# LarissaReames-NOAA/MPASSIT

Hardware: AMD Instinct MI355X
Metric: interpolated 3-D fields/sec (nCells x nLev -> nx x ny) (higher is better)
Workload: dtype f64

## Files before the change

mpassit_amd/build.py:

```python
import os
import subprocess
import sys
from concurrent.futures import ThreadPoolExecutor

HERE = os.path.dirname(os.path.abspath(__file__))
CSRC = os.path.join(HERE, "csrc")
OBJDIR = os.path.join(HERE, "_build")
SO = os.path.join(HERE, "libmpassit_amd.so")
SOURCES = ["mpg_api.hip", "mpg_comm.hip", "mpg_hostpipe.hip", "mpg_fileio.hip", "k_setup.hip", "k_mesh_window.hip", "k_target_grid.hip", "k_store_bilinear.hip", "k_store_nearest.hip", "k_store_conserve.hip",
           "k_store_gridbil.hip", "k_apply.hip", "k_apply_lfu.hip", "k_apply_typed.hip", "k_wind.hip", "k_pole.hip", "k_post.hip", "k_halo.hip", "k_prims.hip", "k_sort.hip", "k_transpose.hip", "k_apply_masked.hip", "k_store_to_mesh.hip", "k_apply_to_mesh.hip", "k_apply_csr_to_mesh.hip", "k_store_mesh.hip", "k_apply_rows.hip",
           "k_store_conserve_mesh.hip", "k_apply_csr_rows.hip", "k_store_periodic_to_mesh.hip"]
HEADERS = ["mpg_internal.h", "geom.h", "quad_solve.h", "conserve_clip.h", "apply_mesh.h", os.path.join("..", "..", "include", "mpassit_amd.h")]
HIPCC = os.environ.get("HIPCC", "/opt/rocm/bin/hipcc")
FLAGS = ["--offload-arch=gfx950", "-O3", "-fPIC", "-std=c++17", "-Wall", "-Wno-unused-function", "-fno-gpu-rdc"]


def _newer(a, deps):
    if not os.path.exists(a):
        return False
    t = os.path.getmtime(a)
    return all(os.path.getmtime(d) <= t for d in deps)


def build(force=False, verbose=False):
    os.makedirs(OBJDIR, exist_ok=True)
    hdrs = [os.path.join(CSRC, h) for h in HEADERS]
    jobs = []
    objs = []
    for s in SOURCES:
        src = os.path.join(CSRC, s)
        obj = os.path.join(OBJDIR, s.replace(".hip", ".o"))
        objs.append(obj)
        if force or not _newer(obj, [src] + hdrs):
            jobs.append([HIPCC] + FLAGS + ["-c", src, "-o", obj])

    def run(cmd):
        if verbose:
            print(" ".join(cmd), flush=True)
        r = subprocess.run(cmd, capture_output=True, text=True)
        if r.returncode != 0:
            raise RuntimeError("hipcc failed:\n%s\n%s" % (" ".join(cmd), r.stderr[-8000:]))
        return r.stderr

    if jobs:
        with ThreadPoolExecutor(max_workers=min(4, len(jobs))) as ex:
# ... 102 lines not shown
```

mpassit_amd/csrc/mpg_api.hip:

```cpp
#include <stdarg.h>
#include <stdio.h>
#include <stdlib.h>
#include <string.h>
#include <time.h>

#include <condition_variable>
#include <deque>
#include <map>
#include <memory>
#include <mutex>
#include <thread>
#include <unordered_map>
#include <vector>

#include "mpg_internal.h"

static thread_local char g_err[1024] = "";
static bool g_init = false;
static int g_device = -1;
static hipStream_t g_stream = nullptr;
static std::map<HandleKey, mpg_handle_s *> g_cache;
#define MPG_MAX_PARKED 8
static uint64_t g_park_clock = 0;
static std::recursive_mutex g_cache_mu;
#define CACHE_LOCK() std::lock_guard<std::recursive_mutex> cache_lock_(g_cache_mu)
static void store_worker_drain();
static void store_worker_stop();
static int store_worker_start(int device);

void mpg_set_error(const char *fmt, ...) {
  va_list ap;
  va_start(ap, fmt);
  vsnprintf(g_err, sizeof(g_err), fmt, ap);
  va_end(ap);
}
bool mpg_is_initialized() { return g_init; }
hipStream_t mpg_setup_stream() { return g_stream; }
int mpg_device_index() { return g_device; }

void mpg_cache_detach(mpg_handle_s *h) {
  CACHE_LOCK();
  if (h->cached) {
    g_cache.erase(h->key);
    h->cached = false;
  }
}

namespace {
struct PoolBlock { void *p; size_t bytes; hipStream_t stream; };
std::vector<PoolBlock> g_pool;
std::mutex g_pool_mu;
size_t g_pool_bytes = 0;
const size_t POOL_CAP_BYTES = (size_t)4 << 30;
}

void *mpg_pool_get(size_t bytes, hipStream_t s) {
  bytes = (bytes + 255) & ~(size_t)255;
  {
    std::lock_guard<std::mutex> lk(g_pool_mu);
    int best = -1;
    for (int i = 0; i < (int)g_pool.size(); ++i) {
      const PoolBlock &b = g_pool[i];
      if (b.stream != s || b.bytes < bytes || b.bytes > 2 * bytes + (1 << 20)) continue;
      if (best < 0 || b.bytes < g_pool[best].bytes) best = i;
    }
    if (best >= 0) {
      void *p = g_pool[best].p;
      g_pool_bytes -= g_pool[best].bytes;
      g_pool.erase(g_pool.begin() + best);
      return p;
    }
  }
  void *p = nullptr;
  hipError_t e = hipMalloc(&p, bytes);
  if (e != hipSuccess) {
    mpg_pool_release();
    e = hipMalloc(&p, bytes);
  }
  if (e != hipSuccess) {
    mpg_set_error("HIP error %s allocating %zu bytes of scratch", hipGetErrorString(e), bytes);
    return nullptr;
  }
  return p;
}

static std::unordered_map<void *, size_t> g_pool_real;

void mpg_pool_put(void *p, size_t bytes, hipStream_t s) {
  if (!p) return;
  bytes = (bytes + 255) & ~(size_t)255;
  std::lock_guard<std::mutex> lk(g_pool_mu);
  auto it = g_pool_real.find(p);
  if (it != g_pool_real.end()) bytes = it->second;
  else g_pool_real[p] = bytes;
  if (g_pool_bytes + bytes > POOL_CAP_BYTES) {
    g_pool_real.erase(p);
    (void)hipFree(p);
    return;
  }
  g_pool.push_back(PoolBlock{p, bytes, s});
  g_pool_bytes += bytes;
}

void mpg_pool_release() {
  std::lock_guard<std::mutex> lk(g_pool_mu);
  for (const PoolBlock &b : g_pool) (void)hipFree(b.p);
  g_pool.clear();
  g_pool_real.clear();
  g_pool_bytes = 0;
}


#define MPG_ANCHORS(X) X(k_setup) X(k_target_grid) X(k_store_bilinear) X(k_store_nearest) X(k_store_conserve) X(k_store_gridbil) \
  X(k_apply) X(k_apply_lfu) X(k_apply_typed) X(k_wind) X(k_pole) X(k_post) X(k_halo) X(mpg_comm) X(k_mesh_window) X(k_prims) X(k_sort) \
  X(k_transpose) X(k_apply_masked) X(k_store_to_mesh) X(k_apply_to_mesh) X(k_apply_csr_to_mesh) \
  X(k_store_mesh) X(k_apply_rows) X(k_store_conserve_mesh) X(k_apply_csr_rows) X(k_store_periodic_to_mesh)
#define X(n) const void *mpg_anchor_##n();
MPG_ANCHORS(X)
#undef X
static std::thread *g_warm = nullptr;
static bool g_init_trace = false;
static double now_ms() {
  struct timespec ts;
  clock_gettime(CLOCK_MONOTONIC, &ts);
  return (double)ts.tv_sec * 1e3 + (double)ts.tv_nsec * 1e-6;
}
static void warm_modules(int device) {
  if (hipSetDevice(device) != hipSuccess) return;
  (void)store_worker_start(device);
  hipFuncAttributes a;
  double t0 = now_ms();
#define X(n)                                                                                                          \
  (void)hipFuncGetAttributes(&a, mpg_anchor_##n());                                                                   \
  if (g_init_trace) {                                                                                                 \
// ... 52 lines not shown
  MPG_ARG(device >= 0 && device < n, "mpg_init: device index out of range");
  if (g_init && device != g_device) {
    mpg_set_error("mpg_init: already initialised on device %d; call mpg_finalize before initialising device %d", g_device, device);
    return MPG_ERR_INVALID_ARG;
  }
  MPG_HIP(hipSetDevice(device));
  const double t_2 = now_ms();
  if (!g_init) {
    MPG_HIP(hipStreamCreateWithFlags(&g_stream, hipStreamNonBlocking));
    if (g_init_trace)
      fprintf(stderr, "mpg_init trace: hipGetDeviceCount (runtime start) %.2f ms, hipSetDevice %.2f ms, stream %.2f ms\n", t_1 - t_0, t_2 - t_1,
              now_ms() - t_2);
    const char *e = getenv("MPG_NO_WARMUP");
    if (!(e && *e == '1')) {
      g_warm = new std::thread(warm_modules, device);
      static bool registered = false;
      if (!registered) {
        atexit(warm_join);
        registered = true;
      }
    }
  }
  g_device = device;
  g_init = true;
  return MPG_SUCCESS;
}

int mpg_warmup_wait(void) {
  warm_join();
  store_worker_drain();
  return MPG_SUCCESS;
}

static void handle_free(mpg_handle_s *h);
static void drop_parked(void *obj) {
  CACHE_LOCK();
  for (auto it = g_cache.begin(); it != g_cache.end();) {
    mpg_handle_s *h = it->second;
    if (h->refcount == 0 && (!obj || std::get<0>(it->first) == obj || std::get<2>(it->first) == obj)) {
      it = g_cache.erase(it);
      handle_free(h);
    } else {
      ++it;
    }
  }
}

int mpg_finalize(void) {
  if (!g_init) return MPG_SUCCESS;
  warm_join();
  store_worker_stop();
  drop_parked(nullptr);
  mpg_fileio_release();
  mpg_hostpipe_release();
  (void)hipStreamSynchronize(g_stream);
  mpg_pool_release();
  (void)hipStreamDestroy(g_stream);
  g_stream = nullptr;
  g_init = false;
  return MPG_SUCCESS;
}

int mpg_device_count(int *n) {
  MPG_ARG(n, "mpg_device_count: NULL argument");
  int c = 0;
  if (hipGetDeviceCount(&c) != hipSuccess) c = 0;
// ... 7 lines not shown
  MPG_HIP(hipGetDeviceProperties(&p, g_device));
  if (arch_buf && buf_len > 0) {
    strncpy(arch_buf, p.gcnArchName, (size_t)buf_len - 1);
    arch_buf[buf_len - 1] = 0;
  }
  if (n_cu) *n_cu = p.multiProcessorCount;
  if (hbm_bytes) *hbm_bytes = (int64_t)p.totalGlobalMem;
  return MPG_SUCCESS;
}

static std::vector<mpg_mesh_s *> g_meshes;

static int mesh_common_checks(int64_t nCells, int64_t nVertices, int maxEdges, const double *latCell, const double *lonCell, const double *latVertex,
                              const double *lonVertex, const int32_t *verticesOnCell, mpg_mesh *out, const char *who) {
  if (!out) { mpg_set_error("%s: out is NULL", who); return MPG_ERR_INVALID_ARG; }
  if (!(nCells > 0 && nVertices > 0 && maxEdges >= 3)) { mpg_set_error("%s: nCells, nVertices must be > 0 and maxEdges >= 3", who); return MPG_ERR_INVALID_ARG; }
  if (!(nCells < 0x7fffffff && nVertices < 0x7fffffff)) { mpg_set_error("%s: sizes must fit int32 ids", who); return MPG_ERR_INVALID_ARG; }
  if (!(latCell && lonCell && latVertex && lonVertex && verticesOnCell)) { mpg_set_error("%s: NULL array", who); return MPG_ERR_INVALID_ARG; }
  return MPG_SUCCESS;
}

int mpg_mesh_create_window(int64_t nCells, int64_t nVertices, int maxEdges, const double *latCell, const double *lonCell, const double *latVertex,
                           const double *lonVertex, const int32_t *verticesOnCell, mpg_grid grid, mpg_mesh *out) {
  MPG_CHECK_INIT();
  int rc = mesh_common_checks(nCells, nVertices, maxEdges, latCell, lonCell, latVertex, lonVertex, verticesOnCell, out, "mpg_mesh_create_window");
  if (rc) return rc;
  MPG_ARG(grid, "mpg_mesh_create_window: NULL grid");
  mpg_mesh_s *m = new mpg_mesh_s();
  m->nCells = nCells;
  m->nVertices = nVertices;
  m->maxEdges = maxEdges;
  m->geo_grid = grid;
  g_meshes.push_back(m);
  if ((rc = mpg_k_mesh_coords(nCells, lonCell, latCell, m->cell, g_stream)) ||
      (rc = mpg_k_mesh_window(m, grid, latVertex, lonVertex, verticesOnCell, g_stream))) {
    mpg_mesh_destroy(m);
    return rc;
  }
  *out = m;
  return MPG_SUCCESS;
}

int mpg_mesh_window_info(mpg_mesh m, int64_t *cell_first, int64_t *cell_count, int64_t *vertex_first, int64_t *vertex_count, double *margin) {
  MPG_ARG(m, "mpg_mesh_window_info: NULL mesh");
  if (cell_first) *cell_first = m->cw0;
  if (cell_count) *cell_count = m->cwn;
  if (vertex_first) *vertex_first = m->vw0;
  if (vertex_count) *vertex_count = m->vwn;
  if (margin) *margin = m->geo_margin;
  return MPG_SUCCESS;
}

int mpg_mesh_create(int64_t nCells, int64_t nVertices, int maxEdges, const double *latCell, const double *lonCell,
                    const double *latVertex, const double *lonVertex, const int32_t *verticesOnCell, mpg_mesh *out) {
  MPG_CHECK_INIT();
  {
    int rc0 = mesh_common_checks(nCells, nVertices, maxEdges, latCell, lonCell, latVertex, lonVertex, verticesOnCell, out, "mpg_mesh_create");
    if (rc0) return rc0;
  }
  mpg_mesh_s *m = new mpg_mesh_s();
  m->nCells = nCells;
  m->nVertices = nVertices;
  m->maxEdges = maxEdges;
  m->cwn = nCells;
  m->vwn = nVertices;
  m->geo_margin = 4.0;
// ... 199 lines not shown
int mpg_grid_get_rotang(mpg_grid g, double *cosa_host, double *sina_host) {
  const double *c, *s;
  int rc = mpg_grid_rotang_dev(g, &c, &s);
  if (rc) return rc;
  size_t bytes = sizeof(double) * (size_t)g->nx * g->ny;
  if (cosa_host) MPG_HIP(hipMemcpy(cosa_host, c, bytes, hipMemcpyDeviceToHost));
  if (sina_host) MPG_HIP(hipMemcpy(sina_host, s, bytes, hipMemcpyDeviceToHost));
  return MPG_SUCCESS;
}

static void handle_free(mpg_handle_s *h) {
  h->idx.free();
  h->w.free();
  h->rowptr.free();
  h->col.free();
  h->val.free();
  h->dst_frac.free();
  h->pole_dst.free();
  h->pole_src0.free();
  h->pole_w.free();
  h->free_tile_lists();
  delete h;
}

struct StoreCtx {
  mpg_mesh_s *m;
  mpg_grid_s *g;
  int stagger;
  int method;
  int meshloc;
  mpg_mesh_s *dst_mesh = nullptr;
};

struct StoreJob {
  HandleKey key;
  int (*build)(mpg_handle_s *, void *, hipStream_t);
  StoreCtx ctx;
  hipEvent_t ready = nullptr;
  bool done = false;
  int rc = MPG_SUCCESS;
  char err[1024] = "";
  ~StoreJob() {
    if (ready) (void)hipEventDestroy(ready);
  }
};
struct StoreWorker {
  std::mutex mu, start_mu;
  std::condition_variable cv;
  std::deque<std::shared_ptr<StoreJob>> queue;
  std::map<HandleKey, std::shared_ptr<StoreJob>> pending;
  std::thread *thread = nullptr;
  hipStream_t stream = nullptr;
  bool stop = false;
};
static StoreWorker &SW() {
  static StoreWorker *w = new StoreWorker();
  return *w;
}
static const char *mpg_last_error_cstr() { return g_err; }

static int store_build_now(StoreJob &job, hipStream_t s) {
  mpg_handle_s *h = new mpg_handle_s();
  h->refcount = 0;
  hipEvent_t e0 = nullptr, e1 = nullptr;
  if (hipEventCreate(&e0) != hipSuccess || hipEventCreate(&e1) != hipSuccess) {
    mpg_set_error("hipEventCreate failed in a RegridStore");
    handle_free(h);
    return MPG_ERR_HIP;
  }
  (void)hipEventRecord(e0, s);
  int rc = job.build(h, &job.ctx, s);
  if (!rc) {
    hipError_t e = hipEventRecord(e1, s);
    if (e == hipSuccess) e = hipEventSynchronize(e1);
    if (e == hipSuccess) e = hipEventElapsedTime(&h->store_ms, e0, e1);
    if (e != hipSuccess) {
      mpg_set_error("RegridStore: %s", hipGetErrorString(e));
      rc = MPG_ERR_HIP;
    }
  }
  (void)hipEventDestroy(e0);
  (void)hipEventDestroy(e1);
  if (rc) {
    handle_free(h);
    return rc;
  }
  CACHE_LOCK();
  h->key = job.key;
  h->cached = true;
  h->parked_at = ++g_park_clock;
  g_cache[job.key] = h;
  return MPG_SUCCESS;
}

static void store_worker_main(int device) {
  const hipError_t dev_err = hipSetDevice(device);
  for (;;) {
    std::shared_ptr<StoreJob> job;
    {
      std::unique_lock<std::mutex> lk(SW().mu);
      SW().cv.wait(lk, [] { return SW().stop || !SW().queue.empty(); });
      if (SW().queue.empty()) return;
      job = SW().queue.front();
      SW().queue.pop_front();
    }
    g_err[0] = 0;
    int rc;
    if (dev_err != hipSuccess) {
      mpg_set_error("RegridStore: the Store worker could not bind device %d: %s", device, hipGetErrorString(dev_err));
      rc = MPG_ERR_HIP;
    } else {
      if (job->ready) (void)hipStreamWaitEvent(SW().stream, job->ready, 0);
      rc = store_build_now(*job, SW().stream);
    }
    {
      std::lock_guard<std::mutex> lk(SW().mu);
      job->rc = rc;
      if (rc) snprintf(job->err, sizeof(job->err), "%s", mpg_last_error_cstr());
      job->done = true;
      SW().pending.erase(job->key);
    }
    SW().cv.notify_all();
  }
}

static int store_worker_start(int device) {
  std::lock_guard<std::mutex> lk(SW().start_mu);
  if (SW().thread) return MPG_SUCCESS;
  MPG_HIP(hipStreamCreateWithFlags(&SW().stream, hipStreamNonBlocking));
  SW().stop = false;
  SW().thread = new std::thread(store_worker_main, device);
  return MPG_SUCCESS;
}

static void store_worker_drain() {
  std::unique_lock<std::mutex> lk(SW().mu);
  SW().cv.wait(lk, [] { return SW().pending.empty(); });
}

static void store_worker_stop() {
  if (!SW().thread) return;
  store_worker_drain();
  {
    std::lock_guard<std::mutex> lk(SW().mu);
    SW().stop = true;
  }
  SW().cv.notify_all();
  SW().thread->join();
  delete SW().thread;
  SW().thread = nullptr;
  (void)hipStreamDestroy(SW().stream);
  SW().stream = nullptr;
}

static int store_common(HandleKey key, mpg_handle *out, int (*build)(mpg_handle_s *, void *, hipStream_t), const StoreCtx &ctx) {
  for (int attempt = 0; attempt < 2; ++attempt) {
    {
      CACHE_LOCK();
      auto it = g_cache.find(key);
      if (it != g_cache.end()) {
        if (out) {
          it->second->refcount++;
          *out = it->second;
        }
        return MPG_SUCCESS;
      }
    }
    int rc = store_worker_start(g_device);
    if (rc) return rc;
    std::shared_ptr<StoreJob> job;
    {
      std::unique_lock<std::mutex> lk(SW().mu);
      auto pit = SW().pending.find(key);
      if (pit != SW().pending.end()) {
        job = pit->second;
      } else {
        job = std::make_shared<StoreJob>();
        job->key = key;
        job->build = build;
        job->ctx = ctx;
        if (hipEventCreateWithFlags(&job->ready, hipEventDisableTiming) == hipSuccess) (void)hipEventRecord(job->ready, g_stream);
        SW().pending[key] = job;
        SW().queue.push_back(job);
      }
      if (!out) {
        lk.unlock();
        SW().cv.notify_all();
        return MPG_SUCCESS;
      }
      SW().cv.notify_all();
      SW().cv.wait(lk, [&] { return job->done; });
    }
    if (job->rc) {
      mpg_set_error("%s", job->err);
      return job->rc;
    }
  }
  mpg_set_error("RegridStore: the finished handle left the cache before it was collected");
  return MPG_ERR_HIP;
}

static int store_mesh_build(mpg_handle_s *h, void *c, hipStream_t s) {
  StoreCtx *x = (StoreCtx *)c;
  h->method = x->method;
  int rc;
  if (x->method == MPG_REGRIDMETHOD_BILINEAR) rc = mpg_k_store_bilinear_mesh(x->m, x->g, x->stagger, x->meshloc, h, s);
  else if (x->method == MPG_REGRIDMETHOD_NEAREST_STOD) rc = mpg_k_store_nearest(x->m, x->g, x->stagger, h, s);
  else rc = mpg_k_store_conserve(x->m, x->g, h, s);
  if (!rc && x->m->win_count[x->meshloc] >= 0)
    rc = mpg_k_rebase(h, x->m->win_first[x->meshloc], x->m->win_count[x->meshloc], s, true);
  return rc;
}
static int store_grid_build(mpg_handle_s *h, void *c, hipStream_t s) {
  StoreCtx *x = (StoreCtx *)c;
  h->method = x->method;
  return mpg_k_store_grid_bilinear(x->g, x->stagger, h, s);
}

static int store_mesh_entry(mpg_mesh src, int src_meshloc, mpg_grid dst, int dst_staggerloc, int regridmethod, mpg_handle *out, const char *who) {
  MPG_CHECK_INIT();
  MPG_ARG(src && dst, "mpg_regrid_store: NULL argument");
  MPG_ARG(dst_staggerloc >= 0 && dst_staggerloc <= 2, "mpg_regrid_store: destination stagger must be CENTER, EDGE1 or EDGE2");
  MPG_ARG(src_meshloc == MPG_MESHLOC_ELEMENT || src_meshloc == MPG_MESHLOC_NODE, "mpg_regrid_store: unknown mesh location");
  if (src_meshloc == MPG_MESHLOC_NODE && regridmethod != MPG_REGRIDMETHOD_BILINEAR) {
    mpg_set_error("%s: node-located sources are only regridded bilinearly by the reference (interp.F90:350-366)", who);
    return MPG_ERR_UNSUPPORTED;
  }
  MPG_ARG(regridmethod >= 0 && regridmethod <= 2, "mpg_regrid_store: unknown regrid method");
  if (src->geo_grid && (src->geo_grid != dst || src->geo_grid_gone)) {
    mpg_set_error("%s: the mesh was cut to another grid (mpg_mesh_create_window%s); it holds only the cells that grid can see", who,
                  src->geo_grid_gone ? ", which has been destroyed" : "");
    return MPG_ERR_INVALID_ARG;
  }
  if (regridmethod == MPG_REGRIDMETHOD_CONSERVE && dst_staggerloc != MPG_STAGGERLOC_CENTER) {
    mpg_set_error("%s: conservative regridding is defined on the CENTER stagger only", who);
    return MPG_ERR_UNSUPPORTED;
  }
  StoreCtx ctx{src, dst, dst_staggerloc, regridmethod, src_meshloc};
  HandleKey key(src, src_meshloc, dst, dst_staggerloc,
                regridmethod + (regridmethod == MPG_REGRIDMETHOD_BILINEAR ? 16 * mpg_bilinear_linetype() : 0) +
                    (regridmethod == MPG_REGRIDMETHOD_BILINEAR && src_meshloc == MPG_MESHLOC_NODE ? 256 * (mpg_node_fan_origin() + 16) : 0));
  return store_common(key, out, store_mesh_build, ctx);
}

int mpg_regrid_store(mpg_mesh src, int src_meshloc, mpg_grid dst, int dst_staggerloc, int regridmethod, mpg_handle *out) {
  MPG_CHECK_INIT();
  MPG_ARG(out, "mpg_regrid_store: NULL argument");
  return store_mesh_entry(src, src_meshloc, dst, dst_staggerloc, regridmethod, out, "mpg_regrid_store");
}
int mpg_regrid_store_begin(mpg_mesh src, int src_meshloc, mpg_grid dst, int dst_staggerloc, int regridmethod) {
  return store_mesh_entry(src, src_meshloc, dst, dst_staggerloc, regridmethod, nullptr, "mpg_regrid_store_begin");
}

int mpg_handle_source_range(mpg_handle h, int64_t *first, int64_t *end) {
  MPG_CHECK_INIT();
  MPG_ARG(h && first && end, "mpg_handle_source_range: NULL argument");
  MPG_ARG(!h->localized, "mpg_handle_source_range: the handle was re-indexed (mpg_handle_localize / mpg_handle_rebase)");
  int rc = mpg_k_source_range(h, first, end, g_stream);
  if (rc) return rc;
  if (h->cached && std::get<1>(h->key) < 100) {
    mpg_mesh_s *m = (mpg_mesh_s *)std::get<0>(h->key);
    const int loc = std::get<1>(h->key);
    if (m->win_count[loc] >= 0 && *end > *first) {
      *first += m->win_first[loc];
      *end += m->win_first[loc];
    }
  }
  return MPG_SUCCESS;
}

int mpg_mesh_set_source_window(mpg_mesh m, int meshloc, int64_t first, int64_t count) {
  MPG_CHECK_INIT();
  MPG_ARG(m && (meshloc == MPG_MESHLOC_ELEMENT || meshloc == MPG_MESHLOC_NODE), "mpg_mesh_set_source_window: bad mesh / location");
  const int64_t n_all = meshloc == MPG_MESHLOC_ELEMENT ? m->nCells : m->nVertices;
  MPG_ARG(first >= 0 && count >= 0 && first + count <= n_all, "mpg_mesh_set_source_window: the window must lie inside the mesh");
// ... 6 lines not shown
    int64_t f = 0, e = 0;
    int rc = mpg_k_source_range(kv.second, &f, &e, g_stream);
    if (rc) return rc;
    if (e > f && (f + old_first < first || e + old_first > first + count)) {
      mpg_set_error("mpg_mesh_set_source_window: a route handle of this mesh references sources [%lld, %lld), outside the window [%lld, %lld)",
                    (long long)(f + old_first), (long long)(e + old_first), (long long)first, (long long)(first + count));
      return MPG_ERR_INVALID_ARG;
    }
  }
  for (auto &kv : g_cache) {
    if (std::get<0>(kv.first) != (void *)m || std::get<1>(kv.first) != meshloc) continue;
    mpg_handle_s *h = kv.second;
    h->free_tile_lists();
    h->lf_choice = 0;
    h->cf_choice = 0;
    int rc = mpg_k_rebase(h, first - old_first, count, g_stream, true);
    if (rc) return rc;
  }
  m->win_first[meshloc] = first;
  m->win_count[meshloc] = first == 0 && count == n_all ? -1 : count;
  return MPG_SUCCESS;
}

static int store_grid_entry(mpg_grid grid, int src_staggerloc, int dst_staggerloc, int regridmethod, mpg_handle *out) {
  MPG_CHECK_INIT();
  MPG_ARG(grid, "mpg_regrid_store_grid: NULL argument");
  if (src_staggerloc != MPG_STAGGERLOC_CENTER || (dst_staggerloc != MPG_STAGGERLOC_EDGE1 && dst_staggerloc != MPG_STAGGERLOC_EDGE2) ||
      regridmethod != MPG_REGRIDMETHOD_BILINEAR) {
    mpg_set_error("mpg_regrid_store_grid: only bilinear CENTER -> EDGE1/EDGE2 is used by the reference (interp.F90:298,316)");
    return MPG_ERR_UNSUPPORTED;
  }
  StoreCtx ctx{nullptr, grid, dst_staggerloc, regridmethod, 0};
  HandleKey key(grid, 100 + src_staggerloc, grid, dst_staggerloc, regridmethod + 256 * mpg_grid_inside_tol_exp());
  return store_common(key, out, store_grid_build, ctx);
}
int mpg_regrid_store_grid(mpg_grid grid, int src_staggerloc, int dst_staggerloc, int regridmethod, mpg_handle *out) {
  MPG_CHECK_INIT();
  MPG_ARG(out, "mpg_regrid_store_grid: NULL argument");
  return store_grid_entry(grid, src_staggerloc, dst_staggerloc, regridmethod, out);
}
int mpg_regrid_store_grid_begin(mpg_grid grid, int src_staggerloc, int dst_staggerloc, int regridmethod) {
  return store_grid_entry(grid, src_staggerloc, dst_staggerloc, regridmethod, nullptr);
}

#define MPG_KEY_TO_MESH (1 << 20)
static int store_to_mesh_build(mpg_handle_s *h, void *c, hipStream_t s) {
  StoreCtx *x = (StoreCtx *)c;
  h->method = x->method;
  return mpg_k_store_to_mesh(x->g, x->stagger, x->m, x->meshloc, x->method, h, s);
}

int mpg_regrid_store_to_mesh(mpg_grid src, int src_staggerloc, mpg_mesh dst, int dst_meshloc, int regridmethod, mpg_handle *out) {
  MPG_CHECK_INIT();
  MPG_ARG(src && dst && out, "mpg_regrid_store_to_mesh: NULL argument");
  MPG_ARG(src_staggerloc >= MPG_STAGGERLOC_CENTER && src_staggerloc <= MPG_STAGGERLOC_CORNER, "mpg_regrid_store_to_mesh: unknown stagger location");
  MPG_ARG(dst_meshloc == MPG_MESHLOC_ELEMENT || dst_meshloc == MPG_MESHLOC_NODE, "mpg_regrid_store_to_mesh: unknown mesh location");
  MPG_ARG(regridmethod >= 0 && regridmethod <= 2, "mpg_regrid_store_to_mesh: unknown regrid method");
  if (regridmethod == MPG_REGRIDMETHOD_CONSERVE) {
    mpg_set_error("mpg_regrid_store_to_mesh: conservative Grid -> Mesh regridding is not supported (bilinear and nearest are). "
                  "mpg_regrid_store_conserve_to_mesh is the conservative Store, with its normalisation argument.");
    return MPG_ERR_UNSUPPORTED;
  }
  if (regridmethod == MPG_REGRIDMETHOD_BILINEAR && (src->periodic & MPG_GRID_PERIODIC_I)) {
    mpg_set_error("mpg_regrid_store_to_mesh: bilinear from a periodic grid (MPG_GRID_PERIODIC_I: the i-wrap and the pole caps) is not supported; "
                  "nearest is, and mpg_regrid_store_periodic_to_mesh is the bilinear Store of such a grid, with its pole method argument");
    return MPG_ERR_UNSUPPORTED;
  }
  if (dst->geo_grid) {
    mpg_set_error("mpg_regrid_store_to_mesh: the mesh was cut to a grid (mpg_mesh_create_window): its resident cells are a window and the result "
                  "would be a partial mesh");
    return MPG_ERR_UNSUPPORTED;
  }
  const int64_t n_src = (int64_t)src->snx[src_staggerloc] * src->sny[src_staggerloc];
  const int64_t n_dst = dst_meshloc == MPG_MESHLOC_ELEMENT ? dst->nCells : dst->nVertices;
  if (n_src > 0x7fffffffLL || n_dst > 0x7fffffffLL) {
    mpg_set_error("mpg_regrid_store_to_mesh: %lld source points / %lld mesh points exceed int32 ids", (long long)n_src, (long long)n_dst);
    return MPG_ERR_OVERFLOW;
  }
  if (src->pts[src_staggerloc].n != n_src) {
    mpg_set_error("mpg_regrid_store_to_mesh: the grid holds no coordinates of stagger %d", src_staggerloc);
    return MPG_ERR_INVALID_ARG;
  }
  StoreCtx ctx{dst, src, src_staggerloc, regridmethod, dst_meshloc};
  HandleKey key(src, 200 + src_staggerloc, dst, dst_meshloc,
                regridmethod + (regridmethod == MPG_REGRIDMETHOD_BILINEAR ? 256 * mpg_grid_inside_tol_exp() : 0) + MPG_KEY_TO_MESH);
  return store_common(key, out, store_to_mesh_build, ctx);
}

#define MPG_KEY_PERIODIC (1 << 22)
static int store_periodic_to_mesh_build(mpg_handle_s *h, void *c, hipStream_t s) {
  StoreCtx *x = (StoreCtx *)c;
  h->method = MPG_REGRIDMETHOD_BILINEAR;
  return mpg_k_store_periodic_to_mesh(x->g, x->m, x->meshloc, x->method, h, s);
}

int mpg_regrid_store_periodic_to_mesh(mpg_grid src, mpg_mesh dst, int dst_meshloc, int pole_method, mpg_handle *out) {
  MPG_CHECK_INIT();
  MPG_ARG(src && dst && out, "mpg_regrid_store_periodic_to_mesh: NULL argument");
  MPG_ARG(dst_meshloc == MPG_MESHLOC_ELEMENT || dst_meshloc == MPG_MESHLOC_NODE,
          "mpg_regrid_store_periodic_to_mesh: unknown mesh location (MPG_MESHLOC_ELEMENT or MPG_MESHLOC_NODE)");
  MPG_ARG(pole_method == MPG_POLEMETHOD_NONE || pole_method == MPG_POLEMETHOD_ALLAVG,
          "mpg_regrid_store_periodic_to_mesh: pole_method must be MPG_POLEMETHOD_NONE or MPG_POLEMETHOD_ALLAVG (NPNTAVG and TEETH are not built)");
  if (!(src->periodic & MPG_GRID_PERIODIC_I)) {
    mpg_set_error("mpg_regrid_store_periodic_to_mesh: the grid was not created with MPG_GRID_PERIODIC_I; mpg_regrid_store_to_mesh is the "
                  "Store of a regional grid");
    return MPG_ERR_UNSUPPORTED;
  }
  if (dst->geo_grid) {
    mpg_set_error("mpg_regrid_store_periodic_to_mesh: the mesh was cut to a grid (mpg_mesh_create_window): its resident cells are a window and "
                  "the result would be a partial mesh; create the whole mesh with mpg_mesh_create");
    return MPG_ERR_UNSUPPORTED;
  }
  if (src->nx < 3 || src->ny < 2) {
    mpg_set_error("mpg_regrid_store_periodic_to_mesh: a periodic bilinear Store needs nx >= 3 and ny >= 2 CENTER points, not %d x %d", src->nx,
                  src->ny);
    return MPG_ERR_INVALID_ARG;
  }
  const int64_t n_src = (int64_t)src->nx * src->ny;
  const int64_t n_dst = dst_meshloc == MPG_MESHLOC_ELEMENT ? dst->nCells : dst->nVertices;
  if (n_src > 0x7fffffffLL || n_dst > 0x7fffffffLL) {
    mpg_set_error("mpg_regrid_store_periodic_to_mesh: %lld source points / %lld mesh points exceed int32 ids", (long long)n_src, (long long)n_dst);
    return MPG_ERR_OVERFLOW;
  }
  if (src->pts[MPG_STAGGERLOC_CENTER].n != n_src) {
    mpg_set_error("mpg_regrid_store_periodic_to_mesh: the grid holds no CENTER coordinates");
    return MPG_ERR_INVALID_ARG;
  }
  StoreCtx ctx{dst, src, MPG_STAGGERLOC_CENTER, pole_method, dst_meshloc};
  HandleKey key(src, 200 + MPG_STAGGERLOC_CENTER, dst, dst_meshloc,
                MPG_REGRIDMETHOD_BILINEAR + 256 * mpg_grid_inside_tol_exp() + 65536 * pole_method + MPG_KEY_TO_MESH + MPG_KEY_PERIODIC);
  return store_common(key, out, store_periodic_to_mesh_build, ctx);
}

static int store_conserve_to_mesh_build(mpg_handle_s *h, void *c, hipStream_t s) {
  StoreCtx *x = (StoreCtx *)c;
  h->method = MPG_REGRIDMETHOD_CONSERVE;
  return mpg_k_store_conserve_to_mesh(x->g, x->m, x->method, h, s);
}

int mpg_regrid_store_conserve_to_mesh(mpg_grid src, mpg_mesh dst, int norm_type, mpg_handle *out) {
  MPG_CHECK_INIT();
  MPG_ARG(src && dst && out, "mpg_regrid_store_conserve_to_mesh: NULL argument");
  MPG_ARG(norm_type == MPG_NORM_DSTAREA || norm_type == MPG_NORM_FRACAREA,
          "mpg_regrid_store_conserve_to_mesh: norm_type must be MPG_NORM_DSTAREA or MPG_NORM_FRACAREA");
  if (dst->geo_grid) {
    mpg_set_error("mpg_regrid_store_conserve_to_mesh: the mesh was cut to a grid (mpg_mesh_create_window): its resident cells are a window and the "
                  "result would be a partial mesh");
    return MPG_ERR_UNSUPPORTED;
  }
  if (dst->nCells > 0x7fffffffLL || (int64_t)src->nx * src->ny > 0x7fffffffLL) {
    mpg_set_error("mpg_regrid_store_conserve_to_mesh: %lld grid cells / %lld mesh cells exceed int32 ids", (long long)src->nx * src->ny,
                  (long long)dst->nCells);
    return MPG_ERR_OVERFLOW;
  }
  StoreCtx ctx{dst, src, MPG_STAGGERLOC_CENTER, norm_type, MPG_MESHLOC_ELEMENT};
  HandleKey key(src, 200 + MPG_STAGGERLOC_CENTER, dst, MPG_MESHLOC_ELEMENT, MPG_REGRIDMETHOD_CONSERVE + 256 * norm_type + MPG_KEY_TO_MESH);
  return store_common(key, out, store_conserve_to_mesh_build, ctx);
}

#define MPG_KEY_MESH_MESH (1 << 21)
static int store_mesh_mesh_build(mpg_handle_s *h, void *c, hipStream_t s) {
  StoreCtx *x = (StoreCtx *)c;
  h->method = x->method;
  int rc = mpg_k_store_mesh(x->m, x->dst_mesh, x->stagger, x->method, h, s);
  if (!rc && x->m->win_count[MPG_MESHLOC_ELEMENT] >= 0)
    rc = mpg_k_rebase(h, x->m->win_first[MPG_MESHLOC_ELEMENT], x->m->win_count[MPG_MESHLOC_ELEMENT], s, true);
  return rc;
}

int mpg_regrid_store_mesh(mpg_mesh src, int src_meshloc, mpg_mesh dst, int dst_meshloc, int regridmethod, mpg_handle *out) {
  MPG_CHECK_INIT();
  MPG_ARG(src && dst && out, "mpg_regrid_store_mesh: NULL argument");
  MPG_ARG(src_meshloc == MPG_MESHLOC_ELEMENT || src_meshloc == MPG_MESHLOC_NODE, "mpg_regrid_store_mesh: unknown source mesh location");
  MPG_ARG(dst_meshloc == MPG_MESHLOC_ELEMENT || dst_meshloc == MPG_MESHLOC_NODE, "mpg_regrid_store_mesh: unknown destination mesh location");
  MPG_ARG(regridmethod >= 0 && regridmethod <= 2, "mpg_regrid_store_mesh: unknown regrid method");
  if (regridmethod == MPG_REGRIDMETHOD_CONSERVE) {
    mpg_set_error("mpg_regrid_store_mesh: conservative Mesh -> Mesh regridding is not supported (bilinear and nearest are): the clip of "
                  "Voronoi cell against Voronoi cell is not built.  Two hops through a grid (mpg_regrid_store with MPG_REGRIDMETHOD_CONSERVE, "
                  "then mpg_regrid_store_conserve_to_mesh) are the conservative route today.  mpg_regrid_store_conserve_mesh is the "
                  "conservative Mesh -> Mesh Store, with its normalisation argument.");
    return MPG_ERR_UNSUPPORTED;
  }
  if (src_meshloc == MPG_MESHLOC_NODE) {
    mpg_set_error("mpg_regrid_store_mesh: node-located sources are not supported (the fan triangulation onto a mesh is not built); "
                  "sources are the cell centres, MPG_MESHLOC_ELEMENT -- the destination may be either location");
    return MPG_ERR_UNSUPPORTED;
  }
  if (src->geo_grid || dst->geo_grid) {
    mpg_set_error("mpg_regrid_store_mesh: the %s mesh was cut to a grid (mpg_mesh_create_window): its resident cells are a window; "
                  "create the whole mesh with mpg_mesh_create",
                  src->geo_grid ? "source" : "destination");
    return MPG_ERR_UNSUPPORTED;
  }
  const int64_t n_dst = dst_meshloc == MPG_MESHLOC_ELEMENT ? dst->nCells : dst->nVertices;
  if (src->nCells > 0x7fffffffLL || src->nVertices > 0x7fffffffLL || n_dst > 0x7fffffffLL) {
    mpg_set_error("mpg_regrid_store_mesh: %lld source cells / %lld source triangles / %lld destination points exceed int32 ids",
                  (long long)src->nCells, (long long)src->nVertices, (long long)n_dst);
    return MPG_ERR_OVERFLOW;
  }
  StoreCtx ctx{src, nullptr, dst_meshloc, regridmethod, src_meshloc, dst};
  HandleKey key(src, src_meshloc, dst, dst_meshloc,
                regridmethod + (regridmethod == MPG_REGRIDMETHOD_BILINEAR ? 16 * mpg_bilinear_linetype() : 0) + MPG_KEY_MESH_MESH);
  return store_common(key, out, store_mesh_mesh_build, ctx);
}

static int store_conserve_mesh_build(mpg_handle_s *h, void *c, hipStream_t s) {
  StoreCtx *x = (StoreCtx *)c;
  h->method = MPG_REGRIDMETHOD_CONSERVE;
  int rc = mpg_k_store_conserve_mesh(x->m, x->dst_mesh, x->method, h, s);
  if (!rc && x->m->win_count[MPG_MESHLOC_ELEMENT] >= 0)
    rc = mpg_k_rebase(h, x->m->win_first[MPG_MESHLOC_ELEMENT], x->m->win_count[MPG_MESHLOC_ELEMENT], s, true);
  return rc;
}

int mpg_regrid_store_conserve_mesh(mpg_mesh src, mpg_mesh dst, int norm_type, mpg_handle *out) {
  MPG_CHECK_INIT();
  MPG_ARG(src && dst && out, "mpg_regrid_store_conserve_mesh: NULL argument");
  MPG_ARG(norm_type == MPG_NORM_DSTAREA || norm_type == MPG_NORM_FRACAREA,
          "mpg_regrid_store_conserve_mesh: norm_type must be MPG_NORM_DSTAREA or MPG_NORM_FRACAREA");
  if (src->geo_grid || dst->geo_grid) {
    mpg_set_error("mpg_regrid_store_conserve_mesh: the %s mesh was cut to a grid (mpg_mesh_create_window): its resident cells are a window; "
                  "create the whole mesh with mpg_mesh_create",
                  src->geo_grid ? "source" : "destination");
    return MPG_ERR_UNSUPPORTED;
  }
  if (src->maxEdges > 12 || dst->maxEdges > 12) {
    mpg_set_error("mpg_regrid_store_conserve_mesh: maxEdges %d > 12", src->maxEdges > dst->maxEdges ? src->maxEdges : dst->maxEdges);
    return MPG_ERR_UNSUPPORTED;
  }
  if (src->nCells > 0x7fffffffLL || dst->nCells > 0x7fffffffLL) {
    mpg_set_error("mpg_regrid_store_conserve_mesh: %lld source cells / %lld destination cells exceed int32 ids", (long long)src->nCells,
                  (long long)dst->nCells);
    return MPG_ERR_OVERFLOW;
  }
  StoreCtx ctx{src, nullptr, MPG_MESHLOC_ELEMENT, norm_type, MPG_MESHLOC_ELEMENT, dst};
  HandleKey key(src, MPG_MESHLOC_ELEMENT, dst, MPG_MESHLOC_ELEMENT, MPG_REGRIDMETHOD_CONSERVE + 256 * norm_type + MPG_KEY_MESH_MESH);
  return store_common(key, out, store_conserve_mesh_build, ctx);
}

int mpg_handle_get_dst_frac(mpg_handle h, double *frac_host) {
  MPG_CHECK_INIT();
  MPG_ARG(h && frac_host, "mpg_handle_get_dst_frac: NULL argument");
  MPG_ARG(h->dst_frac.p, "mpg_handle_get_dst_frac: the handle has no destination fraction (mpg_regrid_store_conserve_to_mesh stores one, "
                       "and so does mpg_regrid_store_conserve_mesh)");
  MPG_HIP(hipStreamSynchronize(g_stream));
  if (h->n_dst > 0) MPG_HIP(hipMemcpy(frac_host, h->dst_frac.p, sizeof(double) * (size_t)h->n_dst, hipMemcpyDeviceToHost));
  return MPG_SUCCESS;
}

int mpg_handle_release(mpg_handle h) {
  if (!h) return MPG_SUCCESS;
  CACHE_LOCK();
  if (--h->refcount > 0) return MPG_SUCCESS;
  if (!h->cached) {
    handle_free(h);
    return MPG_SUCCESS;
  }
  h->parked_at = ++g_park_clock;
  int nparked = 0;
  for (auto &kv : g_cache) nparked += kv.second->refcount == 0;
  while (nparked > MPG_MAX_PARKED) {
    auto old = g_cache.end();
    for (auto it = g_cache.begin(); it != g_cache.end(); ++it)
      if (it->second->refcount == 0 && (old == g_cache.end() || it->second->parked_at < old->second->parked_at)) old = it;
    mpg_handle_s *victim = old->second;
    g_cache.erase(old);
    handle_free(victim);
    --nparked;
  }
  return MPG_SUCCESS;
// ... 531 lines not shown
  MPG_ARG(h->n_pole == 0, "mpg_handle_localize: handles with pole terms (periodic Grid -> Grid) cannot be re-indexed");
  MPG_NOT_WINDOWED(h, "mpg_handle_localize");
  if (h->cached) {
    CACHE_LOCK();
    g_cache.erase(h->key);
    h->cached = false;
  }
  std::vector<int32_t> ids;
  lf_invalidate(h);
  return mpg_k_unique_sources(h, ids, true, g_stream);
}

int mpg_handle_rebase(mpg_handle h, int64_t base, int64_t n_local) {
  MPG_CHECK_INIT();
  MPG_ARG(h, "mpg_handle_rebase: NULL handle");
  MPG_ARG(!h->localized, "mpg_handle_rebase: handle already localized");
  MPG_ARG(h->refcount <= 1, "mpg_handle_rebase: the handle is shared (a second mpg_regrid_store returned it from the cache); "
                            "re-indexing it in place would corrupt the other holder's indices -- release the other reference first");
  MPG_ARG(h->n_pole == 0, "mpg_handle_rebase: handles with pole terms (periodic Grid -> Grid) cannot be re-indexed");
  MPG_ARG(base >= 0 && n_local >= 0 && n_local < 0x7fffffff, "mpg_handle_rebase: bad range");
  MPG_NOT_WINDOWED(h, "mpg_handle_rebase");
  if (h->cached) {
    CACHE_LOCK();
    g_cache.erase(h->key);
    h->cached = false;
  }
  lf_invalidate(h);
  return mpg_k_rebase(h, base, n_local, g_stream);
}

int mpg_tune(const char *key, int value) {
  MPG_ARG(key, "mpg_tune: NULL key");
  store_worker_drain();
  int rc = mpg_k_tune(key, value);
  if (rc) mpg_set_error("mpg_tune: unknown key or value out of range: %s=%d", key, value);
  return rc;
}

int mpg_pack_dev(const double *src_dev, int64_t n_src, int nlev, const int32_t *ids_dev, int64_t n_ids, double *dst_dev, void *hip_stream) {
  MPG_CHECK_INIT();
  MPG_ARG(src_dev && ids_dev && dst_dev, "mpg_pack_dev: NULL argument");
  return mpg_k_pack(src_dev, n_src, nlev, ids_dev, n_ids, dst_dev, (hipStream_t)hip_stream);
}

int mpg_dev_alloc(int64_t nbytes, void **out_dev) {
  MPG_CHECK_INIT();
  MPG_ARG(out_dev && nbytes >= 0, "mpg_dev_alloc: bad argument");
  *out_dev = nullptr;
  if (nbytes == 0) return MPG_SUCCESS;
  if (hipMalloc(out_dev, (size_t)nbytes) != hipSuccess) {
    (void)hipGetLastError();
    mpg_release_caches();
    MPG_HIP(hipMalloc(out_dev, (size_t)nbytes));
  }
  return MPG_SUCCESS;
}

int mpg_dev_free(void *dev) {
  MPG_CHECK_INIT();
  if (dev) MPG_HIP(hipFree(dev));
  return MPG_SUCCESS;
}

int mpg_dev_upload(void *dst_dev, const void *src_host, int64_t nbytes) {
  MPG_CHECK_INIT();
  MPG_ARG(nbytes >= 0 && (nbytes == 0 || (dst_dev && src_host)), "mpg_dev_upload: bad argument");
// ... 73 lines not shown
```

Baseline: 2702.

## Run regrid store builds on two worker lanes with conflict guards

Replaces the single background Store worker thread and stream with two lanes, each with its own thread and HIP stream. A job is dispatched to a lane only when its guards (mesh/grid objects and sub-structures) do not conflict with the job running on the other lane, so independent weight builds can overlap. Pool blocks freed on a settled stream become reusable from any stream. This adds scheduling complexity and a risk of races on shared mesh state; mesh creation now drains pending stores first.

```diff
diff --git a/mpassit_amd/build.py b/mpassit_amd/build.py
--- a/mpassit_amd/build.py
+++ b/mpassit_amd/build.py
@@ -10,7 +10,7 @@
 SOURCES = ["mpg_api.hip", "mpg_comm.hip", "mpg_hostpipe.hip", "mpg_fileio.hip", "k_setup.hip", "k_mesh_window.hip", "k_target_grid.hip", "k_store_bilinear.hip", "k_store_nearest.hip", "k_store_conserve.hip",
            "k_store_gridbil.hip", "k_apply.hip", "k_apply_lfu.hip", "k_apply_typed.hip", "k_wind.hip", "k_pole.hip", "k_post.hip", "k_halo.hip", "k_prims.hip", "k_sort.hip", "k_transpose.hip", "k_apply_masked.hip", "k_store_to_mesh.hip", "k_apply_to_mesh.hip", "k_apply_csr_to_mesh.hip", "k_store_mesh.hip", "k_apply_rows.hip",
            "k_store_conserve_mesh.hip", "k_apply_csr_rows.hip", "k_store_periodic_to_mesh.hip"]
-HEADERS = ["mpg_internal.h", "geom.h", "quad_solve.h", "conserve_clip.h", "apply_mesh.h", os.path.join("..", "..", "include", "mpassit_amd.h")]
+HEADERS = ["mpg_internal.h", "geom.h", "quad_solve.h", "conserve_clip.h", "apply_mesh.h", "store_lanes.h", os.path.join("..", "..", "include", "mpassit_amd.h")]
 HIPCC = os.environ.get("HIPCC", "/opt/rocm/bin/hipcc")
 FLAGS = ["--offload-arch=gfx950", "-O3", "-fPIC", "-std=c++17", "-Wall", "-Wno-unused-function", "-fno-gpu-rdc"]
 
diff --git a/mpassit_amd/csrc/mpg_api.hip b/mpassit_amd/csrc/mpg_api.hip
--- a/mpassit_amd/csrc/mpg_api.hip
+++ b/mpassit_amd/csrc/mpg_api.hip
@@ -14,6 +14,7 @@
 #include <vector>
 
 #include "mpg_internal.h"
+#include "store_lanes.h"
 
 static thread_local char g_err[1024] = "";
 static bool g_init = false;
@@ -27,6 +28,7 @@
 static void store_worker_drain();
 static void store_worker_stop();
 static int store_worker_start(int device);
+static int store_worker_unfinished();
 
 void mpg_set_error(const char *fmt, ...) {
   va_list ap;
@@ -48,6 +50,7 @@
 
 namespace {
 struct PoolBlock { void *p; size_t bytes; hipStream_t stream; };
+const hipStream_t POOL_ANY_STREAM = (hipStream_t)(intptr_t)-1;
 std::vector<PoolBlock> g_pool;
 std::mutex g_pool_mu;
 size_t g_pool_bytes = 0;
@@ -61,7 +64,7 @@
     int best = -1;
     for (int i = 0; i < (int)g_pool.size(); ++i) {
       const PoolBlock &b = g_pool[i];
-      if (b.stream != s || b.bytes < bytes || b.bytes > 2 * bytes + (1 << 20)) continue;
+      if ((b.stream != s && b.stream != POOL_ANY_STREAM) || b.bytes < bytes || b.bytes > 2 * bytes + (1 << 20)) continue;
       if (best < 0 || b.bytes < g_pool[best].bytes) best = i;
     }
     if (best >= 0) {
@@ -100,6 +103,12 @@
   }
   g_pool.push_back(PoolBlock{p, bytes, s});
   g_pool_bytes += bytes;
+}
+
+void mpg_pool_settled(hipStream_t s) {
+  std::lock_guard<std::mutex> lk(g_pool_mu);
+  for (PoolBlock &b : g_pool)
+    if (b.stream == s) b.stream = POOL_ANY_STREAM;
 }
 
 void mpg_pool_release() {
@@ -218,6 +227,8 @@
   return MPG_SUCCESS;
 }
 
+int mpg_debug_store_unfinished(void) { return store_worker_unfinished(); }
+
 static void handle_free(mpg_handle_s *h);
 static void drop_parked(void *obj) {
   CACHE_LOCK();
@@ -291,6 +302,7 @@
   m->maxEdges = maxEdges;
   m->geo_grid = grid;
   g_meshes.push_back(m);
+  store_worker_drain();
   if ((rc = mpg_k_mesh_coords(nCells, lonCell, latCell, m->cell, g_stream)) ||
       (rc = mpg_k_mesh_window(m, grid, latVertex, lonVertex, verticesOnCell, g_stream))) {
     mpg_mesh_destroy(m);
@@ -556,10 +568,20 @@
   mpg_mesh_s *dst_mesh = nullptr;
 };
 
+enum {
+  SG_ALL = 0,
+  SG_GRID_PYR = 1,
+  SG_GRID_CELLPYR = 5,
+  SG_GRID_END_POLES = 6,
+  SG_MESH_FAN = 7,
+  SG_MESH_BVH = 8,
+  SG_MESH_VALENCE = 9,
+};
 struct StoreJob {
   HandleKey key;
   int (*build)(mpg_handle_s *, void *, hipStream_t);
   StoreCtx ctx;
+  std::vector<StoreGuard> guards;
   hipEvent_t ready = nullptr;
   bool done = false;
   int rc = MPG_SUCCESS;
@@ -569,13 +591,11 @@
   }
 };
 struct StoreWorker {
-  std::mutex mu, start_mu;
-  std::condition_variable cv;
-  std::deque<std::shared_ptr<StoreJob>> queue;
+  StoreLanes<StoreJob> lanes;
+  std::mutex start_mu;
   std::map<HandleKey, std::shared_ptr<StoreJob>> pending;
-  std::thread *thread = nullptr;
-  hipStream_t stream = nullptr;
-  bool stop = false;
+  hipStream_t stream[MPG_STORE_LANES_MAX] = {nullptr, nullptr};
+  int device = -1;
 };
 static StoreWorker &SW() {
   static StoreWorker *w = new StoreWorker();
@@ -601,6 +621,8 @@
     if (e != hipSuccess) {
       mpg_set_error("RegridStore: %s", hipGetErrorString(e));
       rc = MPG_ERR_HIP;
+    } else {
+      mpg_pool_settled(s);
     }
   }
   (void)hipEventDestroy(e0);
@@ -617,67 +639,56 @@
   return MPG_SUCCESS;
 }
 
-static void store_worker_main(int device) {
-  const hipError_t dev_err = hipSetDevice(device);
-  for (;;) {
-    std::shared_ptr<StoreJob> job;
-    {
-      std::unique_lock<std::mutex> lk(SW().mu);
-      SW().cv.wait(lk, [] { return SW().stop || !SW().queue.empty(); });
-      if (SW().queue.empty()) return;
-      job = SW().queue.front();
-      SW().queue.pop_front();
-    }
-    g_err[0] = 0;
-    int rc;
-    if (dev_err != hipSuccess) {
-      mpg_set_error("RegridStore: the Store worker could not bind device %d: %s", device, hipGetErrorString(dev_err));
-      rc = MPG_ERR_HIP;
-    } else {
-      if (job->ready) (void)hipStreamWaitEvent(SW().stream, job->ready, 0);
-      rc = store_build_now(*job, SW().stream);
-    }
-    {
-      std::lock_guard<std::mutex> lk(SW().mu);
-      job->rc = rc;
-      if (rc) snprintf(job->err, sizeof(job->err), "%s", mpg_last_error_cstr());
-      job->done = true;
-      SW().pending.erase(job->key);
-    }
-    SW().cv.notify_all();
-  }
+static void store_lane_build(StoreJob &job, int lane) {
+  static thread_local int bound = 0;
+  static thread_local hipError_t dev_err = hipSuccess;
+  if (!bound) {
+    dev_err = hipSetDevice(SW().device);
+    bound = dev_err == hipSuccess ? 1 : -1;
+  }
+  g_err[0] = 0;
+  if (bound < 0) {
+    mpg_set_error("RegridStore: the Store worker could not bind device %d: %s", SW().device, hipGetErrorString(dev_err));
+    job.rc = MPG_ERR_HIP;
+  } else {
+    if (job.ready) (void)hipStreamWaitEvent(SW().stream[lane], job.ready, 0);
+    job.rc = store_build_now(job, SW().stream[lane]);
+  }
+  if (job.rc) snprintf(job.err, sizeof(job.err), "%s", mpg_last_error_cstr());
+}
+static void store_lane_finished(StoreJob &job) {
+  job.done = true;
+  SW().pending.erase(job.key);
 }
 
 static int store_worker_start(int device) {
   std::lock_guard<std::mutex> lk(SW().start_mu);
-  if (SW().thread) return MPG_SUCCESS;
-  MPG_HIP(hipStreamCreateWithFlags(&SW().stream, hipStreamNonBlocking));
-  SW().stop = false;
-  SW().thread = new std::thread(store_worker_main, device);
-  return MPG_SUCCESS;
-}
-
-static void store_worker_drain() {
-  std::unique_lock<std::mutex> lk(SW().mu);
-  SW().cv.wait(lk, [] { return SW().pending.empty(); });
+  if (SW().lanes.started()) return MPG_SUCCESS;
+  for (int l = 0; l < MPG_STORE_LANES_MAX; ++l)
+    if (!SW().stream[l]) MPG_HIP(hipStreamCreateWithFlags(&SW().stream[l], hipStreamNonBlocking));
+  SW().device = device;
+  SW().lanes.start(store_lane_build, store_lane_finished);
+  return MPG_SUCCESS;
+}
+
+static void store_worker_drain() { SW().lanes.drain(); }
+static int store_worker_unfinished() {
+  std::lock_guard<std::mutex> lk(SW().lanes.mu);
+  return SW().lanes.unfinished;
 }
 
 static void store_worker_stop() {
-  if (!SW().thread) return;
-  store_worker_drain();
-  {
-    std::lock_guard<std::mutex> lk(SW().mu);
-    SW().stop = true;
-  }
-  SW().cv.notify_all();
-  SW().thread->join();
-  delete SW().thread;
-  SW().thread = nullptr;
-  (void)hipStreamDestroy(SW().stream);
-  SW().stream = nullptr;
-}
-
-static int store_common(HandleKey key, mpg_handle *out, int (*build)(mpg_handle_s *, void *, hipStream_t), const StoreCtx &ctx) {
+  std::lock_guard<std::mutex> lk(SW().start_mu);
+  if (!SW().lanes.started()) return;
+  SW().lanes.stop_and_join();
+  for (int l = 0; l < MPG_STORE_LANES_MAX; ++l) {
+    if (SW().stream[l]) (void)hipStreamDestroy(SW().stream[l]);
+    SW().stream[l] = nullptr;
+  }
+}
+
+static int store_common(HandleKey key, mpg_handle *out, int (*build)(mpg_handle_s *, void *, hipStream_t), const StoreCtx &ctx,
+                        const std::vector<StoreGuard> &guards) {
   for (int attempt = 0; attempt < 2; ++attempt) {
     {
       CACHE_LOCK();
@@ -694,7 +705,7 @@
     if (rc) return rc;
     std::shared_ptr<StoreJob> job;
     {
-      std::unique_lock<std::mutex> lk(SW().mu);
+      std::unique_lock<std::mutex> lk(SW().lanes.mu);
       auto pit = SW().pending.find(key);
       if (pit != SW().pending.end()) {
         job = pit->second;
@@ -703,17 +714,18 @@
         job->key = key;
         job->build = build;
         job->ctx = ctx;
+        job->guards = guards;
         if (hipEventCreateWithFlags(&job->ready, hipEventDisableTiming) == hipSuccess) (void)hipEventRecord(job->ready, g_stream);
         SW().pending[key] = job;
-        SW().queue.push_back(job);
+        SW().lanes.push_locked(job);
       }
       if (!out) {
         lk.unlock();
-        SW().cv.notify_all();
+        SW().lanes.cv.notify_all();
         return MPG_SUCCESS;
       }
-      SW().cv.notify_all();
-      SW().cv.wait(lk, [&] { return job->done; });
+      SW().lanes.cv.notify_all();
+      SW().lanes.cv.wait(lk, [&] { return job->done; });
     }
     if (job->rc) {
       mpg_set_error("%s", job->err);
@@ -764,7 +776,17 @@
   HandleKey key(src, src_meshloc, dst, dst_staggerloc,
                 regridmethod + (regridmethod == MPG_REGRIDMETHOD_BILINEAR ? 16 * mpg_bilinear_linetype() : 0) +
                     (regridmethod == MPG_REGRIDMETHOD_BILINEAR && src_meshloc == MPG_MESHLOC_NODE ? 256 * (mpg_node_fan_origin() + 16) : 0));
-  return store_common(key, out, store_mesh_build, ctx);
+  std::vector<StoreGuard> guards;
+  if (regridmethod == MPG_REGRIDMETHOD_BILINEAR) {
+    guards.push_back(StoreGuard{dst, SG_GRID_PYR + dst_staggerloc});
+    if (src_meshloc == MPG_MESHLOC_NODE) guards.push_back(StoreGuard{src, SG_MESH_FAN});
+  } else if (regridmethod == MPG_REGRIDMETHOD_NEAREST_STOD) {
+    guards.push_back(StoreGuard{src, SG_MESH_BVH});
+  } else {
+    guards.push_back(StoreGuard{dst, SG_GRID_CELLPYR});
+    guards.push_back(StoreGuard{src, SG_MESH_VALENCE});
+  }
+  return store_common(key, out, store_mesh_build, ctx, guards);
 }
 
 int mpg_regrid_store(mpg_mesh src, int src_meshloc, mpg_grid dst, int dst_staggerloc, int regridmethod, mpg_handle *out) {
@@ -837,7 +859,7 @@
   }
   StoreCtx ctx{nullptr, grid, dst_staggerloc, regridmethod, 0};
   HandleKey key(grid, 100 + src_staggerloc, grid, dst_staggerloc, regridmethod + 256 * mpg_grid_inside_tol_exp());
-  return store_common(key, out, store_grid_build, ctx);
+  return store_common(key, out, store_grid_build, ctx, {StoreGuard{grid, SG_GRID_END_POLES}});
 }
 int mpg_regrid_store_grid(mpg_grid grid, int src_staggerloc, int dst_staggerloc, int regridmethod, mpg_handle *out) {
   MPG_CHECK_INIT();
@@ -889,7 +911,7 @@
   StoreCtx ctx{dst, src, src_staggerloc, regridmethod, dst_meshloc};
   HandleKey key(src, 200 + src_staggerloc, dst, dst_meshloc,
                 regridmethod + (regridmethod == MPG_REGRIDMETHOD_BILINEAR ? 256 * mpg_grid_inside_tol_exp() : 0) + MPG_KEY_TO_MESH);
-  return store_common(key, out, store_to_mesh_build, ctx);
+  return store_common(key, out, store_to_mesh_build, ctx, {StoreGuard{src, SG_ALL}, StoreGuard{dst, SG_ALL}});
 }
 
 #define MPG_KEY_PERIODIC (1 << 22)
@@ -934,7 +956,7 @@
   StoreCtx ctx{dst, src, MPG_STAGGERLOC_CENTER, pole_method, dst_meshloc};
   HandleKey key(src, 200 + MPG_STAGGERLOC_CENTER, dst, dst_meshloc,
                 MPG_REGRIDMETHOD_BILINEAR + 256 * mpg_grid_inside_tol_exp() + 65536 * pole_method + MPG_KEY_TO_MESH + MPG_KEY_PERIODIC);
-  return store_common(key, out, store_periodic_to_mesh_build, ctx);
+  return store_common(key, out, store_periodic_to_mesh_build, ctx, {StoreGuard{src, SG_ALL}, StoreGuard{dst, SG_ALL}});
 }
 
 static int store_conserve_to_mesh_build(mpg_handle_s *h, void *c, hipStream_t s) {
@@ -960,7 +982,7 @@
   }
   StoreCtx ctx{dst, src, MPG_STAGGERLOC_CENTER, norm_type, MPG_MESHLOC_ELEMENT};
   HandleKey key(src, 200 + MPG_STAGGERLOC_CENTER, dst, MPG_MESHLOC_ELEMENT, MPG_REGRIDMETHOD_CONSERVE + 256 * norm_type + MPG_KEY_TO_MESH);
-  return store_common(key, out, store_conserve_to_mesh_build, ctx);
+  return store_common(key, out, store_conserve_to_mesh_build, ctx, {StoreGuard{src, SG_ALL}, StoreGuard{dst, SG_ALL}});
 }
 
 #define MPG_KEY_MESH_MESH (1 << 21)
@@ -1006,7 +1028,7 @@
   StoreCtx ctx{src, nullptr, dst_meshloc, regridmethod, src_meshloc, dst};
   HandleKey key(src, src_meshloc, dst, dst_meshloc,
                 regridmethod + (regridmethod == MPG_REGRIDMETHOD_BILINEAR ? 16 * mpg_bilinear_linetype() : 0) + MPG_KEY_MESH_MESH);
-  return store_common(key, out, store_mesh_mesh_build, ctx);
+  return store_common(key, out, store_mesh_mesh_build, ctx, {StoreGuard{src, SG_ALL}, StoreGuard{dst, SG_ALL}});
 }
 
 static int store_conserve_mesh_build(mpg_handle_s *h, void *c, hipStream_t s) {
@@ -1040,7 +1062,7 @@
   }
   StoreCtx ctx{src, nullptr, MPG_MESHLOC_ELEMENT, norm_type, MPG_MESHLOC_ELEMENT, dst};
   HandleKey key(src, MPG_MESHLOC_ELEMENT, dst, MPG_MESHLOC_ELEMENT, MPG_REGRIDMETHOD_CONSERVE + 256 * norm_type + MPG_KEY_MESH_MESH);
-  return store_common(key, out, store_conserve_mesh_build, ctx);
+  return store_common(key, out, store_conserve_mesh_build, ctx, {StoreGuard{src, SG_ALL}, StoreGuard{dst, SG_ALL}});
 }
 
 int mpg_handle_get_dst_frac(mpg_handle h, double *frac_host) {
@@ -1638,6 +1660,14 @@
 int mpg_tune(const char *key, int value) {
   MPG_ARG(key, "mpg_tune: NULL key");
   store_worker_drain();
+  if (!strcmp(key, "store_lanes")) {
+    if (value < 1 || value > MPG_STORE_LANES_MAX) {
+      mpg_set_error("mpg_tune: unknown key or value out of range: %s=%d", key, value);
+      return MPG_ERR_INVALID_ARG;
+    }
+    SW().lanes.set_lanes(value);
+    return MPG_SUCCESS;
+  }
   int rc = mpg_k_tune(key, value);
   if (rc) mpg_set_error("mpg_tune: unknown key or value out of range: %s=%d", key, value);
   return rc;
diff --git a/mpassit_amd/csrc/store_lanes.h b/mpassit_amd/csrc/store_lanes.h
--- /dev/null
+++ b/mpassit_amd/csrc/store_lanes.h
@@ -0,0 +1,118 @@
+#pragma once
+#include <condition_variable>
+#include <deque>
+#include <memory>
+#include <mutex>
+#include <thread>
+#include <vector>
+
+#define MPG_STORE_LANES_MAX 2
+
+struct StoreGuard {
+  const void *obj;
+  int what;
+};
+inline bool store_guards_conflict(const StoreGuard &a, const StoreGuard &b) {
+  return a.obj == b.obj && (a.what == 0 || b.what == 0 || a.what == b.what);
+}
+inline bool store_guards_conflict(const std::vector<StoreGuard> &a, const std::vector<StoreGuard> &b) {
+  for (const StoreGuard &x : a)
+    for (const StoreGuard &y : b)
+      if (store_guards_conflict(x, y)) return true;
+  return false;
+}
+
+template <class Job>
+struct StoreLanes {
+  std::mutex mu;
+  std::condition_variable cv;
+  std::deque<std::shared_ptr<Job>> queue;
+  std::shared_ptr<Job> running[MPG_STORE_LANES_MAX];
+  std::thread *threads[MPG_STORE_LANES_MAX] = {nullptr, nullptr};
+  int lanes = MPG_STORE_LANES_MAX;
+  int unfinished = 0;
+  bool stop = false;
+
+  void push_locked(const std::shared_ptr<Job> &job) {
+    queue.push_back(job);
+    ++unfinished;
+  }
+  std::shared_ptr<Job> take_locked(int lane) {
+    if (lane >= lanes) return nullptr;
+    for (int k = 0; k < lane; ++k)
+      if (!running[k]) return nullptr;
+    for (auto it = queue.begin(); it != queue.end(); ++it) {
+      bool free_of_conflict = true;
+      for (int k = 0; k < MPG_STORE_LANES_MAX; ++k)
+        if (k != lane && running[k] && store_guards_conflict((*it)->guards, running[k]->guards)) free_of_conflict = false;
+      if (!free_of_conflict) continue;
+      std::shared_ptr<Job> job = *it;
+      queue.erase(it);
+      running[lane] = job;
+      return job;
+    }
+    return nullptr;
+  }
+  template <class Build, class Finished>
+  void serve(int lane, Build build, Finished finished) {
+    for (;;) {
+      std::shared_ptr<Job> job;
+      bool more;
+      {
+        std::unique_lock<std::mutex> lk(mu);
+        cv.wait(lk, [&] { return (job = take_locked(lane)) != nullptr || (stop && queue.empty()); });
+        if (!job) return;
+        more = !queue.empty();
+      }
+      if (more) cv.notify_all();
+      build(*job, lane);
+      {
+        std::lock_guard<std::mutex> lk(mu);
+        running[lane] = nullptr;
+        --unfinished;
+        finished(*job);
+      }
+      cv.notify_all();
+    }
+  }
+  void drain() {
+    std::unique_lock<std::mutex> lk(mu);
+    cv.wait(lk, [&] { return unfinished == 0; });
+  }
+  void set_lanes(int n) {
+    {
+      std::lock_guard<std::mutex> lk(mu);
+      lanes = n < 1 ? 1 : n > MPG_STORE_LANES_MAX ? MPG_STORE_LANES_MAX : n;
+    }
+    cv.notify_all();
+  }
+  template <class Build, class Finished>
+  void start(Build build, Finished finished) {
+    std::lock_guard<std::mutex> lk(mu);
+    stop = false;
+    for (int l = 0; l < MPG_STORE_LANES_MAX; ++l)
+      if (!threads[l]) threads[l] = new std::thread([this, l, build, finished] { serve(l, build, finished); });
+  }
+  bool started() {
+    std::lock_guard<std::mutex> lk(mu);
+    return threads[0] != nullptr;
+  }
+  void stop_and_join() {
+    drain();
+    std::thread *t[MPG_STORE_LANES_MAX];
+    {
+      std::lock_guard<std::mutex> lk(mu);
+      stop = true;
+      for (int l = 0; l < MPG_STORE_LANES_MAX; ++l) {
+        t[l] = threads[l];
+        threads[l] = nullptr;
+      }
+    }
+    cv.notify_all();
+    for (int l = 0; l < MPG_STORE_LANES_MAX; ++l)
+      if (t[l]) {
+        t[l]->join();
+        delete t[l];
+      }
+  }
+};
```

After: 2696. No clear change (-0.2%).
